# sanurielf/kvxopt

Measured on AMD Instinct MI355X. Metric: sparse Cholesky factor+solve GF/s, higher is better.
Workload: dtype f64; 1 GPU; 5-pt Laplacian 1000x1000, n=1000000, lower CCS int64, nrhs=1, factor+solve per step; nnz_lower=2998000, lnz=32346403, nsuper=58315, nlevels=18, max_front=1897, parallelism=1 GPU

## Files before the change

### kvxopt_amd/csrc/api.cpp

```cpp
#include "chol_internal.hpp"

#include <algorithm>
#include <chrono>
#include <climits>
#include <cstdio>
#include <cstdlib>
#include <cstring>
#include <stdexcept>
#include <string>
#include <mutex>
#include <vector>

using namespace kvx;

static thread_local std::string g_err;

namespace {
struct LazyRegistry {
    std::mutex mu;
    std::vector<std::shared_future<hipGraphExec_t>> futs;
    ~LazyRegistry()
    {
        std::lock_guard<std::mutex> lk(mu);
        for (auto &f : futs)
// ... 479 lines not shown
        destroy_graphs(F);
        lap("graphs");
        for (hipEvent_t e : F->prof_ev)
            if (e) pool_event_put(e, true);
        for (int i = 0; i < 3; i++) {
            if (F->side[i]) pool_stream_put(F->side[i]);
            if (F->ev_join[i]) pool_event_put(F->ev_join[i], false);
        }
        if (F->d_iperm) (void)pool_free(F->d_iperm);
        if (F->d_inv_ptr) (void)pool_free(F->d_inv_ptr);
        if (F->d_inv_src) (void)pool_free(F->d_inv_src);
        if (F->d_keep) (void)pool_free(F->d_keep);
        if (F->d_flists) (void)pool_free(F->d_flists);
        if (F->d_chain) (void)pool_free(F->d_chain);
        dist_release(F);
        for (void *p : {(void *)F->d_subs, (void *)F->d_subs_f, (void *)F->d_subs_lvl, (void *)F->d_cd_woff, (void *)F->d_lists_sw, (void *)F->d_depth})
            if (p) (void)pool_free(p);
        if (F->ev_fork) pool_event_put(F->ev_fork, false);
        for (hipEvent_t e : F->ev_u)
            if (e) pool_event_put(e, false);
        if (F->ev_ujoin) pool_event_put(F->ev_ujoin, false);
        for (hipEvent_t e : F->ev_lvl)
            if (e) pool_event_put(e, false);
        for (int i = 0; i < 4; i++)
            if (F->ev_pipe[i]) pool_event_put(F->ev_pipe[i], false);
        if (F->ev_in) pool_event_put(F->ev_in, false);
        if (F->ev_out) pool_event_put(F->ev_out, false);
        if (F->stream) pool_stream_put(F->stream);
        lap("streams");
    }
    delete F;
    lap("delete");
}

void kvx_free(void *p) { free(p); }

int kvx_dev_malloc(void **p, int64_t bytes) { HIPCHK(pool_malloc(p, (size_t)std::max<int64_t>(bytes, 1))); return KVX_OK; }
int kvx_dev_free(void *p) { HIPCHK(pool_free(p)); return KVX_OK; }
int kvx_dev_upload(void *dst, const void *src, int64_t bytes) { if (bytes > 0) HIPCHK(hipMemcpy(dst, src, (size_t)bytes, hipMemcpyHostToDevice)); return KVX_OK; }
int kvx_dev_download(void *dst, const void *src, int64_t bytes) { if (bytes > 0) HIPCHK(hipMemcpy(dst, src, (size_t)bytes, hipMemcpyDeviceToHost)); return KVX_OK; }
int kvx_dev_sync(void) { HIPCHK(hipDeviceSynchronize()); return KVX_OK; }
int kvx_dev_trim(void) { pool_release_all(); return KVX_OK; }
int kvx_dev_mem_info(int64_t *free_bytes, int64_t *total_bytes)
{
    size_t f = 0, t = 0;
    HIPCHK(hipMemGetInfo(&f, &t));
// ... 7 lines not shown
```

### kvxopt_amd/csrc/chol_factor.cpp

```cpp
#include "chol_internal.hpp"

#include <algorithm>
#include <climits>
#include <string>

namespace kvx {

int wait_for_caller(kvx_chol *F)
{
    HIPCHK(hipEventRecord(F->ev_in, nullptr));
    HIPCHK(hipStreamWaitEvent(F->stream, F->ev_in, 0));
    return KVX_OK;
}

namespace {

bool dbg_memset_nodes() { return getenv("KVX_DBG_MEMSET_NODES") != nullptr; }

int factor_prologue(kvx_chol *F)
{
    Symbolic &S = F->S;
    hipStream_t st = F->stream;
    const bool nodes = dbg_memset_nodes();
    if (F->d_scptr && !nodes) {
        ProfScope ps(F, FAM_SCATTER);
        launch_init_factor(st, F->d_Ax, F->d_ssrc, F->d_sdst, F->d_scptr, S.lsize, F->d_Lx, F->d_status);
        return KVX_OK;
    }
    if (nodes) {
        HIPCHK(hipMemsetAsync(F->d_Lx, 0, std::max<int64_t>(S.lsize, 1) * sizeof(double), st));
        HIPCHK(hipMemsetAsync(F->d_status, 0x7f, sizeof(int), st));
    } else {
        launch_clear_factor(st, F->d_Lx, S.lsize, F->d_status);
    }
    ProfScope ps(F, FAM_SCATTER);
    launch_scatter_a(st, F->d_Ax, F->d_amap, S.nnzA, F->d_Lx);
    return KVX_OK;
}

int factor_epilogue(kvx_chol *F)
{
    if (F->h_status_dev && !dbg_memset_nodes()) launch_publish_status(F->stream, F->d_status, F->h_status_dev);
    else HIPCHK(hipMemcpyAsync(F->h_status, F->d_status, sizeof(int), hipMemcpyDeviceToHost, F->stream));
    return KVX_OK;
}

int factor_subtree_walk(kvx_chol *F)
{
    hipStream_t st = F->stream;
    const int caps[3] = {32, 48, 64};
    hipStream_t ss[3] = {st, F->side[0], F->side[1]};
    const bool fork[3] = {false, F->nsubf[1] > 0, F->nsubf[2] > 0};
    if (fork[1] || fork[2]) {
        HIPCHK(hipEventRecord(F->ev_fork, st));
        for (int g = 1; g < 3; g++)
            if (fork[g]) HIPCHK(hipStreamWaitEvent(ss[g], F->ev_fork, 0));
    }
    const int64_t offs[3] = {0, F->nsubf[0], F->nsubf[0] + F->nsubf[1]};
    for (int g = 2; g >= 0; g--) {
        if (F->nsubf[g] == 0) continue;
        ProfScope ps(F, FAM_SMALL, ss[g]);
        launch_factor_subtree(ss[g], caps[g], F->ds, F->d_subs_f + offs[g], F->nsubf[g], F->d_depth, F->d_Lx, F->d_U[0], F->d_U[1], F->d_status);
    }
    for (int g = 1; g < 3; g++)
        if (fork[g]) { HIPCHK(hipEventRecord(F->ev_join[g - 1], ss[g])); HIPCHK(hipStreamWaitEvent(st, F->ev_join[g - 1], 0)); }
    return KVX_OK;
}

struct Level {
    kvx_chol *F;
    int l;
    const LevelPlan &P;
    const int32_t *lbase;
    const double *Uch;
    double *Uout;
    const int32_t *list;
    int nbig, bigm;
};

int small_fronts(const Level &L, bool side_used[2])
{
    kvx_chol *F = L.F;
    const LevelPlan &P = L.P;
    hipStream_t st = F->stream;
    const bool have_big = L.nbig > 0;
    struct Item { int c; int cnt; int64_t off; double est; int stream; int mcap; int kmax; };
    Item items[5];
    int nitems = 0;
    for (int c = KVX_CLS_LDS128; c < KVX_CLS_WAVE0; c++)
        if (P.cnt[c] > 0) {
            const double slots = c == KVX_CLS_LDS128 ? 512.0 : 1024.0;
            items[nitems++] = Item{c, P.cnt[c], P.off[c], (P.maxk[c] > 32 ? 80.0 : 45.0) * std::max(1.0, P.cnt[c] / slots), 0, 0, 0};
        }
    for (int c = KVX_CLS_WAVE0; c < KVX_NCLS; c += 2) {
        const int cnt = P.cnt[c] + P.cnt[c + 1];
        if (cnt == 0) continue;
        const int mcap = wave_class_mcap(c);
        const double base = mcap == 64 ? 35.0 : (mcap == 48 ? 28.0 : 18.0), slots = mcap == 64 ? 2048.0 : (mcap == 48 ? 4096.0 : 8192.0);
        items[nitems++] = Item{c, cnt, P.cnt[c] > 0 ? P.off[c] : P.off[c + 1], base * std::max(1.0, cnt / slots), 0, mcap, P.cnt[c] > 0 ? 32 : 16};
    }
// ... 69 lines not shown
{
    kvx_chol *F = L.F;
    hipStream_t st = F->stream;
    ProfScope ps(F, FAM_SYRK);
    if (cls) {
        const kvx_chol::ChainList &cl = F->chain_steps[(size_t)L.l][(size_t)(jb / KVX_NB)];
        launch_syrk_step(st, F->ds, F->d_chain + cl.off, F->chain_m.data() + cl.off, F->chain_k.data() + cl.off, cl.cnt, jb, klen,
                         F->d_Lx, L.Uout, F->d_Linv, F->d_status, col_lim);
    } else if (klen == 2 * KVX_NB) {
        launch_syrk_pair(st, F->ds, L.list, L.nbig, L.bigm, jb, F->d_Lx, L.Uout, F->d_Linv, F->d_status, col_lim);
    } else if (col_lim < KVX_COLS_PIVOT) {
        launch_syrk_inner(st, F->ds, L.list, L.nbig, L.bigm, jb, col_lim, F->d_Lx, L.Uout, F->d_Linv, F->d_status);
    } else {
        launch_syrk_trailing(st, F->ds, L.list, L.nbig, L.bigm, jb, F->d_Lx, L.Uout, F->d_Linv, F->d_status, col_lim);
    }
}

void trsm_step(const Level &L, int jb)
{
    ProfScope ps(L.F, FAM_TRSM);
    launch_trsm_blk(L.F->stream, L.F->ds, L.list, L.nbig, L.bigm, jb, L.F->d_Lx, L.F->d_Linv);
}

void chain_two_level(const Level &L)
{
    kvx_chol *F = L.F;
    hipStream_t st = F->stream;
    const int OB = F->K.outer_block, maxk = L.P.chain_maxk;
    for (int ob = 0; ob < maxk; ob += OB) {
        for (int jb = ob; jb < std::min(ob + OB, maxk); jb += KVX_NB) {
            trsm_step(L, jb);
            { ProfScope ps(F, FAM_SYRK); launch_syrk_inner(st, F->ds, L.list, L.nbig, L.bigm, jb, ob + OB, F->d_Lx, L.Uout, F->d_Linv, F->d_status); }
        }
        { ProfScope ps(F, FAM_SYRK); launch_syrk_outer(st, F->ds, L.list, L.nbig, L.bigm, ob, OB, F->d_Lx, L.Uout, F->d_Linv, F->d_status); }
    }
}

int chain_blocked(const Level &L)
{
    kvx_chol *F = L.F;
    hipStream_t st = F->stream;
    const int OB = F->K.u_block, maxk = L.P.chain_maxk;
    const std::vector<kvx_chol::ChainList> &far = F->u_steps[(size_t)L.l];
    hipStream_t su = (F->K.u_stream && F->prof_family < 0) ? F->side[2] : st;
    bool forked = false;
    for (int ob = 0, b = 0; ob < maxk; ob += OB, b++) {
        const int bend = std::min(ob + OB, maxk);
        for (int jb = ob; jb < bend; jb += KVX_NB) {
            trsm_step(L, jb);
            if (jb + KVX_NB < bend) syrk_step(L, true, jb, KVX_NB, ob + OB);
        }
        const kvx_chol::ChainList &fl = far[(size_t)b];
        if (fl.cnt > 0) {
            if (su != st) {
                while ((int)F->ev_u.size() <= 2 * b + 1) { hipEvent_t e = nullptr; HIPCHK(pool_event_get(&e, false)); F->ev_u.push_back(e); }
                HIPCHK(hipEventRecord(F->ev_u[(size_t)(2 * b)], st));
                HIPCHK(hipStreamWaitEvent(su, F->ev_u[(size_t)(2 * b)], 0));
                forked = true;
                syrk_count(SYRK_FAR_SIDE);
            }
            {
                ProfScope ps(F, FAM_SYRK, su);
                launch_syrk_far(su, F->ds, F->d_chain + fl.off, F->chain_m.data() + fl.off, F->chain_k.data() + fl.off, fl.cnt, ob, OB,
                                ob + 2 * OB, F->d_Lx, L.Uout);
            }
            if (su != st) HIPCHK(hipEventRecord(F->ev_u[(size_t)(2 * b + 1)], su));
        }
        if (bend < maxk) {
            if (su != st && b >= 1 && far[(size_t)(b - 1)].cnt > 0) HIPCHK(hipStreamWaitEvent(st, F->ev_u[(size_t)(2 * (b - 1) + 1)], 0));
            syrk_step(L, true, ob, OB, ob + 2 * OB);
        }
    }
    if (forked) {
        if (!F->ev_ujoin) HIPCHK(pool_event_get(&F->ev_ujoin, false));
        HIPCHK(hipEventRecord(F->ev_ujoin, su));
        HIPCHK(hipStreamWaitEvent(st, F->ev_ujoin, 0));
    }
    return KVX_OK;
}

void chain_pairs(const Level &L, bool cls)
{
    const int maxk = L.P.chain_maxk;
    for (int jb = 0; jb < maxk;) {
        const int64_t T = (L.bigm - jb - 1 + KVX_TILE - 1) / KVX_TILE;
        const bool pair = jb + KVX_NB < maxk && T * (T + 1) / 2 * L.nbig >= L.F->K.pair_tiles;
        trsm_step(L, jb);
        if (!pair) {
            syrk_step(L, cls, jb, KVX_NB, INT_MAX);
            jb += KVX_NB;
            continue;
        }
        syrk_step(L, cls, jb, KVX_NB, jb + 2 * KVX_NB);
        trsm_step(L, jb + KVX_NB);
        syrk_step(L, cls, jb, 2 * KVX_NB, INT_MAX);
        jb += 2 * KVX_NB;
    }
}

int pipe_level_hook(kvx_chol *F, int l)
{
    Symbolic &S = F->S;
    HIPCHK(hipEventRecord(F->ev_lvl[(size_t)l], F->stream));
    hipStream_t sw = F->K.pipe_own_stream ? F->side[2] : F->side[0];
    const SweepStreams ss2{sw, sw, sw, F->ev_pipe[1], F->ev_pipe[2], F->ev_pipe[3]};
    if (l == F->pipe_from) enqueue_fwd(F, F->d_X, S.n, F->pipe_nr, S.nlevels - 1, l, &ss2, true, true);
    else if (l < F->pipe_from) enqueue_fwd(F, F->d_X, S.n, F->pipe_nr, l, l, &ss2, true);
    return KVX_OK;
}

}

int enqueue_factor_body(kvx_chol *F, int lfrom, int lto, bool prologue, bool epilogue)
{
    Symbolic &S = F->S;
    int rc;
    if (prologue && (rc = factor_prologue(F))) return rc;
    if (lfrom < 0) lfrom = S.nlevels - 1;
    if (F->factor_subtrees && prologue && lfrom == S.nlevels - 1 && (rc = factor_subtree_walk(F))) return rc;
    const int32_t *lbase = F->fplan_on ? F->d_flists : F->d_lists;
    for (int l = lfrom; l >= lto; l--) {
        const LevelPlan &P = F->fplan_on ? F->fplan[l] : F->plan[l];
        const Level L{F, l, P, lbase, F->d_U[(l + 1) & 1], F->d_U[l & 1], lbase + P.off[KVX_CLS_BIG], P.cnt[KVX_CLS_BIG], P.maxm[KVX_CLS_BIG]};
        bool side_used[2];
        if ((rc = small_fronts(L, side_used))) return rc;
        if (L.nbig > 0) {
            assemble_big(L);
            const ChainChoice c = choose_chain(P, F->K, have_chain_lists(F, l, P));
            if (c.kind == CHAIN_TWO_LEVEL) chain_two_level(L);
            else if (c.kind == CHAIN_PAIRS) chain_pairs(L, c.cls);
            else if ((rc = chain_blocked(L))) return rc;
        }
        if ((rc = join_small_fronts(F, side_used))) return rc;
        if (F->pipe_on && (rc = pipe_level_hook(F, l))) return rc;
    }
    if (epilogue && (rc = factor_epilogue(F))) return rc;
    HIPCHK(hipGetLastError());
    return KVX_OK;
}

void dump_graph_dot(hipGraph_t graph)
{
    const char *dot = getenv("KVX_DBG_GRAPH_DOT");
    if (!dot) return;
    static int serial = 0;
    const std::string path = std::string(dot) + "." + std::to_string(serial++) + ".dot";
    if (hipGraphDebugDotPrint(graph, path.c_str(), 0) != hipSuccess) (void)hipGetLastError();
}

int enqueue_factor(kvx_chol *F)
{
    if (F->dist_nranks > 1) { set_err("sharded factor: use kvx_chol_dist_factorize"); return KVX_EINVAL; }
    hipStream_t st = F->stream;
    HIPCHK(hipEventRecord(F->ev[0], st));
    const char *dbg_ng = dbg_no_factor_graph();
    const bool graph_ok = F->K.use_graph && F->prof_family < 0 && !(dbg_ng && (atoll(dbg_ng) == 1 || atoll(dbg_ng) == F->S.n));
    F->factor_calls++;
    F->diag_valid = false;
    if (graph_ok && !F->g_factor.tried && F->factor_calls >= 2)
// ... 38 lines not shown
```

### kvxopt_amd/csrc/chol_internal.hpp

```cpp
#pragma once
#include "../../include/kvxhip.h"
#include "abi_guard.hpp"
#include "devpool.hpp"
#include "device.hpp"
#include "symbolic.hpp"

#include <chrono>
#include <cstdint>
#include <cstdlib>
#include <atomic>
#include <future>
#include <string>
#include <vector>

namespace kvx { void set_last_error(const std::string &s); struct DistState; }
#define set_err(s) ::kvx::set_last_error(s)
using namespace kvx;

#define HIPCHK(call)                                                                     \
    do {                                                                                 \
        hipError_t e_ = (call);                                                          \
        if (e_ != hipSuccess) {                                                          \
            set_err(std::string(#call) + ": " + hipGetErrorString(e_));                 \
            return KVX_EDEVICE;                                                          \
// ... 43 lines not shown
        tried = false;
    }
};

struct CholKnobs {
    int sub_maxf = 0;
    bool factor_subtrees = false;
    int u_block = 384;
    bool init_two_passes = false;
    bool use_subtrees = true;
    bool use_graph = true;
    int wide_from = -1;
    int side_spread = 1;
    int two_level_m = 6144;
    int outer_block = 1024;
    int64_t asm_potrf_wgs = 1024;
    int64_t pair_tiles = 3000;
    int defer_u = 1;
    bool syrk_direct = false;
    double blocked_gf = 0.5;
    int u_stream = 1;
    bool pipe_own_stream = false;
    bool solve_nofork = false;
};
CholKnobs read_chol_knobs();
inline const char *dbg_no_factor_graph() { return getenv("KVX_DBG_NO_FACTOR_GRAPH"); }

struct LevelPlan {
    int64_t off[KVX_NCLS];
    int cnt[KVX_NCLS];
    int maxm[KVX_NCLS];
    int maxk[KVX_NCLS];
    int big_maxk = 0;
    int chain_maxk = 0;
    double big_flops = 0.0;
    int64_t soff[3];
    int scnt[3];
    int smaxm[3];
};

struct kvx_chol {
    Symbolic S;
    kvx_chol_opts opts;
    CholKnobs K;
    bool dev_ready = false;
    bool numeric = false;
    bool pending = false;
    bool is_ll = true;
    double *d_diag = nullptr;
    bool diag_valid = false;
    int64_t minor = 0;
    hipStream_t stream = nullptr;
    hipStream_t side[3] = {nullptr, nullptr, nullptr};
    hipEvent_t ev_fork = nullptr, ev_join[3] = {nullptr, nullptr, nullptr};
    hipEvent_t ev_out = nullptr;
    hipEvent_t ev_in = nullptr;
    hipEvent_t ev[4] = {nullptr, nullptr, nullptr, nullptr};
    std::vector<hipEvent_t> ev_lvl;
    bool pipe_on = false;
    int pipe_nr = 0;
    int pipe_from = 0;
    hipEvent_t ev_pipe[4] = {nullptr, nullptr, nullptr, nullptr};
    SubDesc *d_subs_lvl = nullptr;
    std::vector<int> sub_lvl_off, sub_lvl_cnt;
    struct FusedGraph { int nrhs; double *B; int64_t ldB; int calls; LazyExec exec; };
    std::vector<FusedGraph> g_fused;
    bool have_ftime = false, have_stime = false;
    double ms_factor = 0, ms_solve = 0;

    int32_t *d_k = nullptr, *d_m = nullptr, *d_first = nullptr, *d_rowidx = nullptr, *d_rel = nullptr,
            *d_children = nullptr, *d_perm = nullptr, *d_lists = nullptr;
    int64_t *d_px = nullptr, *d_rowptr = nullptr, *d_ux = nullptr, *d_wx = nullptr, *d_childptr = nullptr,
            *d_amap = nullptr, *d_sdst = nullptr, *d_scptr = nullptr;
    double *d_Lx = nullptr, *d_U[2] = {nullptr, nullptr}, *d_Ax = nullptr;
    double *d_X = nullptr, *d_X0 = nullptr, *d_W[2] = {nullptr, nullptr}, *d_WK = nullptr;
    double *d_Linv = nullptr;
    int32_t *d_ssrc = nullptr;
    int64_t scnt = 0;
    int64_t *d_linv_off = nullptr;
    FrontDesc *d_fd = nullptr;
    ChildDesc *d_cd = nullptr;
    int32_t *d_tiles = nullptr;
// ... 82 lines not shown
};
enum { FAM_SCATTER = 0, FAM_SMALL = 1, FAM_ASSEMBLE = 2, FAM_POTRF = 3, FAM_TRSM = 4, FAM_SYRK = 5, FAM_FWD = 6, FAM_BWD = 7 };

inline void prof_collect(kvx_chol *F)
{
    for (size_t i = 0; i + 1 < F->prof_used; i += 2) {
        float ms = 0;
        if (hipEventElapsedTime(&ms, F->prof_ev[i], F->prof_ev[i + 1]) == hipSuccess) { F->prof_ms += ms; F->prof_launches++; }
    }
    F->prof_used = 0;
}


void build_plan_from(const Symbolic &S, const std::vector<int32_t> &lists, const std::vector<int64_t> &lptr, std::vector<LevelPlan> &plan);
void build_plan(kvx_chol *F);
int build_subtrees(kvx_chol *F);
int build_chain_lists(kvx_chol *F);
int ensure_device(kvx_chol *F);
int ensure_solve_ws(kvx_chol *F, int64_t nrhs);
int ensure_wide(kvx_chol *F);
void destroy_graphs(kvx_chol *F);
int wait_for_caller(kvx_chol *F);
int enqueue_factor_body(kvx_chol *F, int lfrom = -1, int lto = 0, bool prologue = true, bool epilogue = true);
int enqueue_factor(kvx_chol *F);
int finish_factor(kvx_chol *F, int64_t *minor);
void dump_graph_dot(hipGraph_t graph);
struct SweepStreams { hipStream_t main, lds, wave; hipEvent_t fork, join0, join1; };
void enqueue_fwd(kvx_chol *F, double *X, int64_t ldx, int nrhs, int lfrom = -1, int lto = 0, const SweepStreams *ss = nullptr, bool wait_levels = false,
                 bool sub_tail = false);
void enqueue_bwd(kvx_chol *F, double *X, int64_t ldx, int nrhs, int lfrom = 0, int lto = -1);
int solve_dev(kvx_chol *F, int sys, double *B, int64_t nrhs, int64_t ldB, bool async = false);
int factor_solve_dev(kvx_chol *F, const double *values_dev, double *B, int64_t nrhs, int64_t ldB, bool async = false);
int spsolve_forward_reach(kvx_chol *F, int sys, int64_t ncol, const int64_t *Bp, const int64_t *Bi, const double *Bx,
                          std::vector<int64_t> &xp, std::vector<int64_t> &xi, std::vector<double> &xx);
void dist_release(kvx_chol *F);

template <class Body>
void capture_graph(kvx_chol *F, Body body, LazyExec &out)
{
    out.tried = true;
    hipGraph_t graph = nullptr;
    if (hipStreamBeginCapture(F->stream, hipStreamCaptureModeRelaxed) != hipSuccess) { (void)hipGetLastError(); return; }
    int rc = body();
    hipError_t e = hipStreamEndCapture(F->stream, &graph);
    if (rc != KVX_OK || e != hipSuccess || !graph) { (void)hipGetLastError(); if (graph) (void)hipGraphDestroy(graph); return; }
    dump_graph_dot(graph);
// ... 19 lines not shown
```

### kvxopt_amd/csrc/chol_setup.cpp

```cpp
#include "chol_internal.hpp"

#include <algorithm>
#include <climits>
#include <vector>

namespace kvx {

bool syrk_direct() { static const bool v = [] { const char *e = getenv("KVX_SYRK_DIRECT"); return e && e[0] == '1'; }(); return v; }

CholKnobs read_chol_knobs()
{
    CholKnobs K;
    const char *e;
    auto is1 = [](const char *v) { return v && v[0] == '1'; };
    if ((e = getenv("KVX_SUB_MAXF"))) K.sub_maxf = std::max(1, std::min(atoi(e), KVX_SUB_MAXF));
    K.factor_subtrees = is1(getenv("KVX_FACTOR_SUBTREES"));
    if ((e = getenv("KVX_U_BLOCK"))) K.u_block = std::max(64, atoi(e) / 64 * 64);
    K.init_two_passes = getenv("KVX_INIT_TWO_PASSES") != nullptr;
    K.use_subtrees = !is1(getenv("KVX_NO_SUBTREES"));
    K.use_graph = !is1(getenv("KVX_NO_GRAPH"));
    if ((e = getenv("KVX_WIDE_FROM"))) K.wide_from = std::max(0, atoi(e));
    if ((e = getenv("KVX_SIDE_SPREAD"))) K.side_spread = atoi(e);
    if ((e = getenv("KVX_TWO_LEVEL_M"))) K.two_level_m = atoi(e);
    if ((e = getenv("KVX_OUTER_BLOCK")) && atoi(e) >= 64) K.outer_block = atoi(e) / 64 * 64;
    if ((e = getenv("KVX_ASM_POTRF_WGS"))) K.asm_potrf_wgs = atoll(e);
    if ((e = getenv("KVX_PAIR_TILES"))) K.pair_tiles = atoll(e);
    if ((e = getenv("KVX_DEFER_U"))) K.defer_u = atoi(e);
    K.syrk_direct = syrk_direct();
    if ((e = getenv("KVX_BLOCKED_GF"))) K.blocked_gf = atof(e);
    if ((e = getenv("KVX_U_STREAM"))) K.u_stream = atoi(e);
    K.pipe_own_stream = is1(getenv("KVX_PIPE_OWN_STREAM"));
    K.solve_nofork = (e = getenv("KVX_SOLVE_NOFORK")) && atoi(e) != 0;
    return K;
}

void build_plan_from(const Symbolic &S, const std::vector<int32_t> &lists, const std::vector<int64_t> &lptr, std::vector<LevelPlan> &plan)
{
    plan.assign((size_t)S.nlevels, LevelPlan());
    for (int l = 0; l < S.nlevels; l++) {
        LevelPlan &P = plan[l];
        for (int c = 0; c < KVX_NCLS; c++) { P.off[c] = 0; P.cnt[c] = 0; P.maxm[c] = 0; P.maxk[c] = 0; }
        for (int g = 0; g < 3; g++) { P.soff[g] = 0; P.scnt[g] = 0; P.smaxm[g] = 0; }
        for (int64_t q = lptr[l]; q < lptr[l + 1]; q++) {
            int s = lists[q];
            int m = S.sn_m[s], k = S.sn_k[s];
            int c = front_class(m, k);
            if (P.cnt[c] == 0) P.off[c] = q;
            P.cnt[c]++;
            P.maxm[c] = std::max(P.maxm[c], m);
            P.maxk[c] = std::max(P.maxk[c], k);
            if (c == KVX_CLS_BIG) {
                P.big_maxk = std::max(P.big_maxk, k);
                P.chain_maxk = std::max(P.chain_maxk, k);
                P.big_flops += (double)k * k * k / 3.0 + (double)(m - k) * k * (double)m;
            }
// ... 395 lines not shown
```

### kvxopt_amd/csrc/chol_solve.cpp

```cpp
#include "chol_internal.hpp"

#include <algorithm>
#include <chrono>
#include <climits>
#include <cstdio>
#include <vector>

namespace kvx {

struct LevelStreams {
    SweepStreams S;
    hipStream_t lds, wave;
    bool fork_lds, fork_wave;
    static SweepStreams own(kvx_chol *F)
    {
        if (F->K.solve_nofork) return SweepStreams{F->stream, F->stream, F->stream, F->ev_fork, F->ev_join[0], F->ev_join[1]};
        return SweepStreams{F->stream, F->side[0], F->side[1], F->ev_fork, F->ev_join[0], F->ev_join[1]};
    }
    LevelStreams(kvx_chol *F, bool have_big, bool have_lds, bool have_wave, const SweepStreams *ss = nullptr) : S(ss ? *ss : own(F))
    {
        fork_lds = have_lds && (have_big || have_wave) && S.lds != S.main;
        fork_wave = have_wave && have_big && S.wave != S.main;
        lds = fork_lds ? S.lds : S.main;
        wave = fork_wave ? S.wave : S.main;
// ... 316 lines not shown
        for (auto &e : F->ev_lvl) HIPCHK(pool_event_get(&e, false));
        for (int i = 0; i < 4; i++) HIPCHK(pool_event_get(&F->ev_pipe[i], false));
        if (F->nsub > 0) {
            std::vector<std::vector<SubDesc>> by((size_t)S.nlevels);
            for (const SubDesc &d : F->subs_host) by[(size_t)S.depth[(size_t)d.hi]].push_back(d);
            std::vector<SubDesc> flat;
            F->sub_lvl_off.assign((size_t)S.nlevels, 0);
            F->sub_lvl_cnt.assign((size_t)S.nlevels, 0);
            for (int l = 0; l < S.nlevels; l++) {
                F->sub_lvl_off[(size_t)l] = (int)flat.size();
                F->sub_lvl_cnt[(size_t)l] = (int)by[(size_t)l].size();
                flat.insert(flat.end(), by[(size_t)l].begin(), by[(size_t)l].end());
            }
            if (F->d_subs_lvl) { (void)pool_free(F->d_subs_lvl); F->d_subs_lvl = nullptr; }
            if ((rc = upload(&F->d_subs_lvl, flat))) return rc;
        }
        int lim = 4;
        if (const char *e = getenv("KVX_PIPE_FRONTS")) lim = atoi(e);
        F->pipe_from = 0;
        for (int l = 0; l < S.nlevels; l++) {
            if (S.levelptr[(size_t)l + 1] - S.levelptr[(size_t)l] > lim) break;
            F->pipe_from = l;
        }
    }
    lap("pipeline set-up");
    hipStream_t st = F->stream, s2 = F->K.pipe_own_stream ? F->side[2] : F->side[0];
    auto body = [&]() -> int {
        HIPCHK(hipEventRecord(F->ev_pipe[0], st));
        HIPCHK(hipStreamWaitEvent(s2, F->ev_pipe[0], 0));
        launch_perm_gather(s2, F->d_perm, n, nr, B, ldB, F->d_X, n);
        launch_copy_d(s2, F->d_X0, F->d_X, n * (int64_t)nr);
        F->pipe_on = true;
        F->pipe_nr = nr;
        const int rb = enqueue_factor_body(F);
        F->pipe_on = false;
        if (rb) return rb;
        HIPCHK(hipEventRecord(F->ev_pipe[0], s2));
        HIPCHK(hipStreamWaitEvent(st, F->ev_pipe[0], 0));
        enqueue_bwd(F, F->d_X, n, nr);
        launch_perm_scatter(st, F->d_perm, n, nr, F->d_X, n, B, ldB);
        return hipGetLastError() == hipSuccess ? KVX_OK : KVX_EDEVICE;
    };
    HIPCHK(hipEventRecord(F->ev[0], st));
    F->factor_calls++;
    F->diag_valid = false;
    kvx_chol::FusedGraph *slot = nullptr;
    if (F->K.use_graph && !dbg_no_factor_graph() && !getenv("KVX_FUSED_EAGER")) {
        for (auto &g : F->g_fused)
            if (g.nrhs == nr && g.B == B && g.ldB == ldB) slot = &g;
        if (!slot) {
            if (F->g_fused.size() >= 4) {
                for (auto &g : F->g_fused) g.exec.drop();
                F->g_fused.clear();
            }
            F->g_fused.push_back({nr, B, ldB, 0, LazyExec{}});
            slot = &F->g_fused.back();
        }
    }
    if ((rc = capture_or_replay(F, slot, true, body))) return rc;
    lap("capture, graph launch or eager enqueue");
    HIPCHK(hipEventRecord(F->ev[1], st));
    HIPCHK(hipGetLastError());
    F->pending = true;
// ... 174 lines not shown
```

### kvxopt_amd/csrc/device.hpp

```cpp
#pragma once
#include <hip/hip_runtime.h>
#include <cstdint>
#include <utility>

namespace kvx {

struct DevSym {
    const int32_t *k;
    const int32_t *m;
    const int32_t *first;
    const int64_t *px;
    const int64_t *rowptr;
    const int32_t *rowidx;
    const int32_t *rel;
    const int64_t *ux;
    const int64_t *wx;
    const int64_t *childptr;
    const int32_t *children;
    const int64_t *linv;
    const struct FrontDesc *fd;
    const struct ChildDesc *cd;
    const int32_t *tiles;
    double piv_floor, piv_repl;
};
// ... 170 lines not shown
void launch_fwd_level(hipStream_t st, const DevSym &ds, const int32_t *list, int count, int max_m,
                      const double *Lx, double *X, int64_t ldx, int nrhs,
                      const double *Wchild, double *Wout, int64_t wstride);
void launch_bwd_level(hipStream_t st, const DevSym &ds, const int32_t *list, int count, int max_m,
                      const double *Lx, double *X, int64_t ldx, int nrhs);
void launch_fwd_wave(hipStream_t st, const DevSym &ds, const int32_t *list, int count, int kmax,
                     const double *Lx, double *X, int64_t ldx, int nrhs, const double *Wchild, double *Wout, int64_t wstride);
void launch_bwd_wave(hipStream_t st, const DevSym &ds, const int32_t *list, int count, int mcap, int kmax,
                     const double *Lx, double *X, int64_t ldx, int nrhs);
void launch_fwd_subtree(hipStream_t st, const DevSym &ds, const SubDesc *subs, int nsub, const int32_t *edges,
                        const double *Lx, double *X, int64_t ldx, int nrhs, double *W0, double *W1, int64_t wstride,
                        const int32_t *depth);
void launch_bwd_subtree(hipStream_t st, const DevSym &ds, const SubDesc *subs, int nsub, int nsub32, const double *Lx, double *X,
                        int64_t ldx, int nrhs);
void launch_bwd_subtree_group(hipStream_t st, int mcap, const DevSym &ds, const SubDesc *subs, int count, const double *Lx, double *X,
                              int64_t ldx);
void launch_fwd_lds(hipStream_t st, const DevSym &ds, const int32_t *list, int count, int kmax,
                    const double *Lx, double *X, int64_t ldx, int nrhs, const double *Wchild, double *Wout, int64_t wstride);
void launch_bwd_lds(hipStream_t st, const DevSym &ds, const int32_t *list, int count,
                    const double *Lx, double *X, int64_t ldx, int nrhs);
void launch_fwd_big(hipStream_t st, const DevSym &ds, const int32_t *list, int count, int max_m, int max_k,
                    const double *Lx, const double *Linv, double *X, const double *X0, int64_t ldx, int nrhs,
                    double *WK, int64_t ldw, const double *Wchild, double *Wout, int64_t wstride, int level_count = 0);
void launch_bwd_big(hipStream_t st, const DevSym &ds, const int32_t *list, int count, int max_m, int max_k,
                    const double *Lx, const double *Linv, double *X, int64_t ldx, int nrhs, double *WK, int64_t ldw);
void launch_perm_gather(hipStream_t st, const int32_t *perm, int64_t n, int nrhs, const double *in, int64_t ldi,
                        double *out, int64_t ldo);
void launch_perm_scatter(hipStream_t st, const int32_t *perm, int64_t n, int nrhs, const double *in, int64_t ldi,
                         double *out, int64_t ldo);
void launch_wide_gather(hipStream_t st, const int32_t *iperm, int64_t n, int nrhs, const double *B, int64_t ldB, double *XT,
                        const double *diag, int mode);
void launch_wide_scatter(hipStream_t st, const int32_t *iperm, int64_t n, int nrhs, const double *XT, double *B, int64_t ldB,
                         const double *diag, int mode);
void launch_wide_fwd_small(hipStream_t st, const DevSym &ds, const int32_t *list, int count, int kmax, int nchunk, const double *Lx,
                           double *XT, int64_t n, const double *Wch, double *Wout, int64_t wstride, const int32_t *inv_ptr,
                           const int32_t *inv_src);
void launch_wide_bwd_small(hipStream_t st, const DevSym &ds, const int32_t *list, int count, int kmax, int nchunk, const double *Lx,
                           double *XT, int64_t n);
void launch_wide_fwd_big(hipStream_t st, const DevSym &ds, const int32_t *list, int count, int max_m, int max_k, int nchunk,
                         const double *Lx, const double *Linv, double *XT, int64_t n, const double *Wch, double *Wout,
                         int64_t wstride, const int32_t *inv_ptr, const int32_t *inv_src);
void launch_wide_bwd_big(hipStream_t st, const DevSym &ds, const int32_t *list, int count, int max_k, int nchunk, const double *Lx,
                         const double *Linv, double *XT, int64_t n);
void launch_zero_slots(hipStream_t st, const int64_t *slots, int count, int nrhs, double *W, int64_t wstride);
void launch_scatter_entries(hipStream_t st, const int64_t *pos, const double *val, int64_t count, double *X);
void launch_mask_rows(hipStream_t st, const uint8_t *keep, int64_t n, int nrhs, double *X, int64_t ldx);
// ... 5 lines not shown
```

### kvxopt_amd/csrc/kernels_big.hip

```cpp
#include "device.hpp"
#include "tile_classes.hpp"

#include <algorithm>
#include <atomic>
#include <climits>
#include <cstdint>
#include <cstdlib>
#include <type_traits>
#include <utility>

namespace kvx {

typedef double d4 __attribute__((ext_vector_type(4)));

#ifdef KVX_PHASE_TIMING
__device__ unsigned long long g_phase[16];
#define KVX_STAMP(var) const unsigned long long var = __builtin_readcyclecounter()
#define KVX_PHASE_ADD(slot, a, b) do { if (threadIdx.x == 0) atomicAdd(&g_phase[slot], (unsigned long long)((b) - (a))); } while (0)
#else
#define KVX_STAMP(var) do { } while (0)
#define KVX_PHASE_ADD(slot, a, b) do { } while (0)
#endif
constexpr int NB = KVX_NB;

// ... 979 lines not shown
    syrk_count(SYRK_T64_GRID);
    hipLaunchKernelGGL(k_syrk_trailing<64>, dim3(T, TC, (unsigned)count), dim3(256), 0, st, ds, list, jb, Lx, Uout, Linv, status, ob_end, no_classes());
}

void launch_syrk_outer(hipStream_t st, const DevSym &ds, const int32_t *list, int count, int max_m, int ob, int ob_len,
                       double *Lx, double *Uout, double *Linv, int *status)
{
    if (count <= 0) return;
    int rows = max_m - ob - 1;
    if (rows <= 0) return;
    syrk_count(SYRK_OUTER);
    hipLaunchKernelGGL(k_syrk_trailing128<false>, syrk128_grid(rows, count), dim3(512), 0, st, ds, list, ob, ob_len, Lx, Uout, Linv, status, ColOwner{1, 1, 0, 0, INT_MAX, 0});
}

void launch_syrk_outer_dist(hipStream_t st, const DevSym &ds, const int32_t *list, int max_m, int ob, int ob_len,
                            int own_ob, int own_g, int own_r, int c_from, int c_to, double *Lx, double *Uout)
{
    int rows = max_m - ob - 1;
    if (rows <= 0 || c_from >= c_to) return;
    hipLaunchKernelGGL(k_syrk_trailing128<true>, syrk128_grid(rows, 1), dim3(512), 0, st, ds, list, ob, ob_len, Lx, Uout,
                       (double *)nullptr, (int *)nullptr, ColOwner{own_ob, own_g, own_r, c_from, c_to, 0});
}

constexpr int SB = 256;
constexpr int SOLVE_NT = 1024;

__device__ __forceinline__ constexpr int sblk(int ib, int s) { return ib * (ib - 1) / 2 + s; }

template <bool FIRST, int ROWS>
__global__ __launch_bounds__(SOLVE_NT) void k_fwd_big_step(DevSym ds, const int32_t *__restrict__ list, int jb0,
                                                           const double *__restrict__ Lx, const double *__restrict__ Linv,
                                                           double *__restrict__ X, const double *__restrict__ X0, int64_t ldx,
                                                           double *__restrict__ WK, int64_t ldw,
                                                           const double *__restrict__ Wc,
                                                           double *__restrict__ Wo, int64_t wstride)
{
    unsigned bx, by, rh;
    kvx_part_front_rhs(bx, by, rh);
    __shared__ double red[3 * 16 * NB];
    __shared__ double own[FIRST ? ROWS : 1];
    __shared__ double wsh[SB];
    __shared__ double ysh[SB];
    const FrontDesc fd = ds.fd[list[by]];
    const int k = fd.k, m = fd.m, f = fd.first, tid = threadIdx.x;
    if (jb0 >= k) return;
    const int nb = min(SB, k - jb0);
    const int rbase = jb0 + nb + bx * ROWS;
// ... 543 lines not shown
#pragma unroll
        for (int c = 0; c < 4; c++)
#pragma unroll
            for (int j = 0; j < 4; j++)
                v[c][j] = kvx_ld0(P, (int64_t)(jb0 + lane + j * NB) + (int64_t)(c0 + c) * m, lane + j * NB < nb && c0 + c < jb0);
#pragma unroll
        for (int b = 0; b < RB; b++) {
            if (b < nv) {
                double a[4] = {0.0, 0.0, 0.0, 0.0};
#pragma unroll
                for (int c = 0; c < 4; c++)
#pragma unroll
                    for (int j = 0; j < 4; j++) a[c] = __builtin_fma(v[c][j], xsh[b][lane + j * NB], a[c]);
                const double u = wave_sum4(a[0], a[1], a[2], a[3], lane);
                if (lane < 4 && c0 + o < jb0) WK[(int64_t)(r0 + b) * ldw + f + c0 + o] -= u;
            }
        }
    }
}

constexpr int KVX_BIG_RB = 8;
constexpr int KVX_BIG_MR_FROM = 64;

void launch_fwd_big(hipStream_t st, const DevSym &ds, const int32_t *list, int count, int max_m, int max_k,
                    const double *Lx, const double *Linv, double *X, const double *X0, int64_t ldx, int nrhs,
                    double *WK, int64_t ldw, const double *Wchild, double *Wout, int64_t wstride, int level_count)
{
    if (count <= 0 || nrhs <= 0) return;
    static const int narrow_wgs = [] { const char *e = getenv("KVX_FWD_NARROW_WGS"); return e ? atoi(e) : 512; }();
    if (nrhs >= KVX_BIG_MR_FROM) {
        for (int jb = 0; jb < max_k; jb += SB) {
            int rows = max_m - jb - 1;
            if ((int64_t)std::max(1, (rows + 63) / 64) * std::max(level_count, count) <= narrow_wgs) {
                dim3 grid((unsigned)std::max(1, (rows + 63) / 64), (unsigned)count, (unsigned)nrhs);
                if (jb == 0) hipLaunchKernelGGL((k_fwd_big_step<true, 64>), grid, dim3(SOLVE_NT), 0, st, ds, list, jb, Lx, Linv, X, X0, ldx, WK, ldw, Wchild, Wout, wstride);
                else hipLaunchKernelGGL((k_fwd_big_step<false, 64>), grid, dim3(SOLVE_NT), 0, st, ds, list, jb, Lx, Linv, X, X0, ldx, WK, ldw, Wchild, Wout, wstride);
                continue;
            }
            const unsigned gz = (unsigned)((nrhs + KVX_BIG_RB - 1) / KVX_BIG_RB);
            dim3 g1(1, (unsigned)count, gz), g2((unsigned)std::max(1, (rows + 255) / 256), (unsigned)count, gz);
            if (jb == 0) {
                hipLaunchKernelGGL((k_fwd_big_step_mr<true, KVX_BIG_RB, 1>), g1, dim3(SOLVE_NT), 0, st, ds, list, jb, Lx, Linv, X, X0, ldx, nrhs, WK, ldw, Wchild, Wout, wstride);
                hipLaunchKernelGGL((k_fwd_big_step_mr<true, KVX_BIG_RB, 2>), g2, dim3(SOLVE_NT), 0, st, ds, list, jb, Lx, Linv, X, X0, ldx, nrhs, WK, ldw, Wchild, Wout, wstride);
            } else {
                hipLaunchKernelGGL((k_fwd_big_step_mr<false, KVX_BIG_RB, 1>), g1, dim3(SOLVE_NT), 0, st, ds, list, jb, Lx, Linv, X, X0, ldx, nrhs, WK, ldw, Wchild, Wout, wstride);
                hipLaunchKernelGGL((k_fwd_big_step_mr<false, KVX_BIG_RB, 2>), g2, dim3(SOLVE_NT), 0, st, ds, list, jb, Lx, Linv, X, X0, ldx, nrhs, WK, ldw, Wchild, Wout, wstride);
            }
        }
        return;
    }
    for (int jb = 0; jb < max_k; jb += SB) {
        int rows = max_m - jb - 1;
        const int64_t wg64 = (int64_t)std::max(1, (rows + 63) / 64) * std::max(level_count, count);
        const bool narrow = wg64 <= narrow_wgs;
        dim3 grid((unsigned)std::max(1, narrow ? (rows + 63) / 64 : (rows + 255) / 256), (unsigned)count, (unsigned)nrhs);
        if (jb == 0) {
            if (narrow) hipLaunchKernelGGL((k_fwd_big_step<true, 64>), grid, dim3(SOLVE_NT), 0, st, ds, list, jb, Lx, Linv, X, X0, ldx, WK, ldw, Wchild, Wout, wstride);
            else hipLaunchKernelGGL((k_fwd_big_step<true, 256>), grid, dim3(SOLVE_NT), 0, st, ds, list, jb, Lx, Linv, X, X0, ldx, WK, ldw, Wchild, Wout, wstride);
        } else {
            if (narrow) hipLaunchKernelGGL((k_fwd_big_step<false, 64>), grid, dim3(SOLVE_NT), 0, st, ds, list, jb, Lx, Linv, X, X0, ldx, WK, ldw, Wchild, Wout, wstride);
            else hipLaunchKernelGGL((k_fwd_big_step<false, 256>), grid, dim3(SOLVE_NT), 0, st, ds, list, jb, Lx, Linv, X, X0, ldx, WK, ldw, Wchild, Wout, wstride);
        }
    }
}

void launch_bwd_big(hipStream_t st, const DevSym &ds, const int32_t *list, int count, int max_m, int max_k,
                    const double *Lx, const double *Linv, double *X, int64_t ldx, int nrhs, double *WK, int64_t ldw)
{
    if (count <= 0 || nrhs <= 0) return;
    (void)max_m;
    if (nrhs >= KVX_BIG_MR_FROM) {
        const unsigned gz = (unsigned)((nrhs + KVX_BIG_RB - 1) / KVX_BIG_RB);
        hipLaunchKernelGGL((k_bwd_big_init_mr<KVX_BIG_RB>), dim3((unsigned)((max_k + 3) / 4), (unsigned)count, gz), dim3(256), 0, st,
                           ds, list, Lx, X, ldx, nrhs, WK, ldw);
        for (int b = (max_k + SB - 1) / SB - 1; b >= 0; b--) {
            hipLaunchKernelGGL((k_bwd_big_step_mr<KVX_BIG_RB, 1>), dim3(1, (unsigned)count, gz), dim3(SOLVE_NT), 0, st, ds, list, b, Lx, Linv,
                               X, ldx, nrhs, WK, ldw);
            if (b > 0)
                hipLaunchKernelGGL((k_bwd_big_step_mr<KVX_BIG_RB, 2>), dim3((unsigned)(b * SB / NB), (unsigned)count, gz), dim3(SOLVE_NT), 0, st, ds, list, b, Lx, Linv,
                                   X, ldx, nrhs, WK, ldw);
        }
        return;
    }
    hipLaunchKernelGGL(k_bwd_big_init, dim3((unsigned)((max_k + 3) / 4), (unsigned)count, (unsigned)nrhs), dim3(256), 0, st,
                       ds, list, Lx, X, ldx, WK, ldw);
    for (int b = (max_k + SB - 1) / SB - 1; b >= 0; b--) {
// ... 8 lines not shown
```

Baseline: 2318 GF/s.

## Pipeline root-front forward solve per block and defer level sweeps behind factor

Splits the forward solve of the root level into per-256-column block launches, each gated by an event recorded after the matching trsm step of the root factorization. The solve can then start on the side stream while the trailing SYRK updates of the root front are still running. It also defers each level's sweep until after the next level's assembly, and moves the status publish onto the sweep stream. The cost is more events and launches, plus more complex ordering logic that could hurt if the side-stream work competes with factor kernels.

```diff
diff --git a/kvxopt_amd/csrc/api.cpp b/kvxopt_amd/csrc/api.cpp
--- a/kvxopt_amd/csrc/api.cpp
+++ b/kvxopt_amd/csrc/api.cpp
@@ -525,6 +525,9 @@
         if (F->ev_ujoin) pool_event_put(F->ev_ujoin, false);
         for (hipEvent_t e : F->ev_lvl)
             if (e) pool_event_put(e, false);
+        for (hipEvent_t e : F->ev_blk)
+            if (e) pool_event_put(e, false);
+        if (F->ev_stat) pool_event_put(F->ev_stat, false);
         for (int i = 0; i < 4; i++)
             if (F->ev_pipe[i]) pool_event_put(F->ev_pipe[i], false);
         if (F->ev_in) pool_event_put(F->ev_in, false);
diff --git a/kvxopt_amd/csrc/chol_factor.cpp b/kvxopt_amd/csrc/chol_factor.cpp
--- a/kvxopt_amd/csrc/chol_factor.cpp
+++ b/kvxopt_amd/csrc/chol_factor.cpp
@@ -35,13 +35,6 @@
     }
     ProfScope ps(F, FAM_SCATTER);
     launch_scatter_a(st, F->d_Ax, F->d_amap, S.nnzA, F->d_Lx);
-    return KVX_OK;
-}
-
-int factor_epilogue(kvx_chol *F)
-{
-    if (F->h_status_dev && !dbg_memset_nodes()) launch_publish_status(F->stream, F->d_status, F->h_status_dev);
-    else HIPCHK(hipMemcpyAsync(F->h_status, F->d_status, sizeof(int), hipMemcpyDeviceToHost, F->stream));
     return KVX_OK;
 }
 
@@ -76,6 +69,7 @@
     double *Uout;
     const int32_t *list;
     int nbig, bigm;
+    bool blocks;
 };
 
 int small_fronts(const Level &L, bool side_used[2])
@@ -191,6 +185,37 @@
     launch_trsm_blk(L.F->stream, L.F->ds, L.list, L.nbig, L.bigm, jb, L.F->d_Lx, L.F->d_Linv);
 }
 
+hipStream_t sweep_stream(const kvx_chol *F) { return F->K.pipe_own_stream ? F->side[2] : F->side[0]; }
+
+int root_block_flush(kvx_chol *F)
+{
+    const int j = F->pend_blk;
+    if (j < 0) return KVX_OK;
+    F->pend_blk = -1;
+    const Symbolic &S = F->S;
+    const LevelPlan &P = F->plan[0];
+    hipStream_t sw = sweep_stream(F);
+    HIPCHK(hipStreamWaitEvent(sw, F->ev_blk[(size_t)j], 0));
+    launch_fwd_big_step(sw, F->ds, F->d_lists + P.soff[0], P.scnt[0], P.smaxm[0], j * KVX_SOLVE_SB, F->d_Lx, F->d_Linv, F->d_X, F->d_X0, S.n,
+                        F->pipe_nr, F->d_WK, S.n, F->d_W[1], F->d_W[0], std::max(S.wrk_size[0], S.wrk_size[1]), P.scnt[0]);
+    return KVX_OK;
+}
+
+int root_block_hook(const Level &L, int jb)
+{
+    kvx_chol *F = L.F;
+    if (!L.blocks) return KVX_OK;
+    const bool last = jb + KVX_NB >= L.P.chain_maxk;
+    if (!last && (jb + KVX_NB) % KVX_SOLVE_SB != 0) return KVX_OK;
+    if (int rc = root_block_flush(F)) return rc;
+    const int j = jb / KVX_SOLVE_SB;
+    if ((size_t)j >= F->ev_blk.size()) { set_err("root pipeline: block event out of range"); return KVX_EINVAL; }
+    HIPCHK(hipEventRecord(F->ev_blk[(size_t)j], F->stream));
+    F->pend_blk = j;
+    if (!(F->K.pipe_edge_order & 1)) return root_block_flush(F);
+    return KVX_OK;
+}
+
 void chain_two_level(const Level &L)
 {
     kvx_chol *F = L.F;
@@ -217,7 +242,11 @@
         const int bend = std::min(ob + OB, maxk);
         for (int jb = ob; jb < bend; jb += KVX_NB) {
             trsm_step(L, jb);
-            if (jb + KVX_NB < bend) syrk_step(L, true, jb, KVX_NB, ob + OB);
+            if (int rc = root_block_hook(L, jb)) return rc;
+            if (jb + KVX_NB < bend) {
+                syrk_step(L, true, jb, KVX_NB, ob + OB);
+                if (int rc = root_block_flush(F)) return rc;
+            }
         }
         const kvx_chol::ChainList &fl = far[(size_t)b];
         if (fl.cnt > 0) {
@@ -238,8 +267,10 @@
         if (bend < maxk) {
             if (su != st && b >= 1 && far[(size_t)(b - 1)].cnt > 0) HIPCHK(hipStreamWaitEvent(st, F->ev_u[(size_t)(2 * (b - 1) + 1)], 0));
             syrk_step(L, true, ob, OB, ob + 2 * OB);
-        }
-    }
+            if (int rc = root_block_flush(F)) return rc;
+        }
+    }
+    if (int rc = root_block_flush(F)) return rc;
     if (forked) {
         if (!F->ev_ujoin) HIPCHK(pool_event_get(&F->ev_ujoin, false));
         HIPCHK(hipEventRecord(F->ev_ujoin, su));
@@ -248,30 +279,52 @@
     return KVX_OK;
 }
 
-void chain_pairs(const Level &L, bool cls)
+int chain_pairs(const Level &L, bool cls)
 {
     const int maxk = L.P.chain_maxk;
     for (int jb = 0; jb < maxk;) {
         const int64_t T = (L.bigm - jb - 1 + KVX_TILE - 1) / KVX_TILE;
         const bool pair = jb + KVX_NB < maxk && T * (T + 1) / 2 * L.nbig >= L.F->K.pair_tiles;
         trsm_step(L, jb);
+        if (int rc = root_block_hook(L, jb)) return rc;
         if (!pair) {
             syrk_step(L, cls, jb, KVX_NB, INT_MAX);
+            if (int rc = root_block_flush(L.F)) return rc;
             jb += KVX_NB;
             continue;
         }
         syrk_step(L, cls, jb, KVX_NB, jb + 2 * KVX_NB);
+        if (int rc = root_block_flush(L.F)) return rc;
         trsm_step(L, jb + KVX_NB);
+        if (int rc = root_block_hook(L, jb + KVX_NB)) return rc;
         syrk_step(L, cls, jb, 2 * KVX_NB, INT_MAX);
+        if (int rc = root_block_flush(L.F)) return rc;
         jb += 2 * KVX_NB;
     }
-}
-
-int pipe_level_hook(kvx_chol *F, int l)
+    return root_block_flush(L.F);
+}
+
+int pipe_level_sweep(kvx_chol *F, int l);
+int pipe_level_hook(kvx_chol *F, int l, bool swept)
+{
+    HIPCHK(hipEventRecord(F->ev_lvl[(size_t)l], F->stream));
+    if (swept) return KVX_OK;
+    if ((F->K.pipe_edge_order & 2) && l > 0) { F->pend_lvl = l; return KVX_OK; }
+    return pipe_level_sweep(F, l);
+}
+
+int pipe_level_flush(kvx_chol *F)
+{
+    const int l = F->pend_lvl;
+    if (l < 0) return KVX_OK;
+    F->pend_lvl = -1;
+    return pipe_level_sweep(F, l);
+}
+
+int pipe_level_sweep(kvx_chol *F, int l)
 {
     Symbolic &S = F->S;
-    HIPCHK(hipEventRecord(F->ev_lvl[(size_t)l], F->stream));
-    hipStream_t sw = F->K.pipe_own_stream ? F->side[2] : F->side[0];
+    hipStream_t sw = sweep_stream(F);
     const SweepStreams ss2{sw, sw, sw, F->ev_pipe[1], F->ev_pipe[2], F->ev_pipe[3]};
     if (l == F->pipe_from) enqueue_fwd(F, F->d_X, S.n, F->pipe_nr, S.nlevels - 1, l, &ss2, true, true);
     else if (l < F->pipe_from) enqueue_fwd(F, F->d_X, S.n, F->pipe_nr, l, l, &ss2, true);
@@ -280,30 +333,41 @@
 
 }
 
+int factor_epilogue(kvx_chol *F, hipStream_t st)
+{
+    if (F->h_status_dev && !dbg_memset_nodes()) launch_publish_status(st, F->d_status, F->h_status_dev);
+    else HIPCHK(hipMemcpyAsync(F->h_status, F->d_status, sizeof(int), hipMemcpyDeviceToHost, st));
+    return KVX_OK;
+}
+
 int enqueue_factor_body(kvx_chol *F, int lfrom, int lto, bool prologue, bool epilogue)
 {
     Symbolic &S = F->S;
     int rc;
+    F->pend_blk = F->pend_lvl = -1;
     if (prologue && (rc = factor_prologue(F))) return rc;
     if (lfrom < 0) lfrom = S.nlevels - 1;
     if (F->factor_subtrees && prologue && lfrom == S.nlevels - 1 && (rc = factor_subtree_walk(F))) return rc;
     const int32_t *lbase = F->fplan_on ? F->d_flists : F->d_lists;
     for (int l = lfrom; l >= lto; l--) {
         const LevelPlan &P = F->fplan_on ? F->fplan[l] : F->plan[l];
-        const Level L{F, l, P, lbase, F->d_U[(l + 1) & 1], F->d_U[l & 1], lbase + P.off[KVX_CLS_BIG], P.cnt[KVX_CLS_BIG], P.maxm[KVX_CLS_BIG]};
+        Level L{F, l, P, lbase, F->d_U[(l + 1) & 1], F->d_U[l & 1], lbase + P.off[KVX_CLS_BIG], P.cnt[KVX_CLS_BIG], P.maxm[KVX_CLS_BIG], false};
         bool side_used[2];
         if ((rc = small_fronts(L, side_used))) return rc;
         if (L.nbig > 0) {
             assemble_big(L);
+            if (F->pipe_on && (rc = pipe_level_flush(F))) return rc;
             const ChainChoice c = choose_chain(P, F->K, have_chain_lists(F, l, P));
+            L.blocks = F->pipe_on && F->pipe_blocks && l == 0 && c.kind != CHAIN_TWO_LEVEL;
             if (c.kind == CHAIN_TWO_LEVEL) chain_two_level(L);
-            else if (c.kind == CHAIN_PAIRS) chain_pairs(L, c.cls);
-            else if ((rc = chain_blocked(L))) return rc;
+            else if (c.kind == CHAIN_PAIRS) rc = chain_pairs(L, c.cls);
+            else rc = chain_blocked(L);
+            if (rc) return rc;
         }
         if ((rc = join_small_fronts(F, side_used))) return rc;
-        if (F->pipe_on && (rc = pipe_level_hook(F, l))) return rc;
-    }
-    if (epilogue && (rc = factor_epilogue(F))) return rc;
+        if (F->pipe_on && ((rc = pipe_level_flush(F)) || (rc = pipe_level_hook(F, l, L.blocks)))) return rc;
+    }
+    if (epilogue && (rc = factor_epilogue(F, F->stream))) return rc;
     HIPCHK(hipGetLastError());
     return KVX_OK;
 }
diff --git a/kvxopt_amd/csrc/chol_internal.hpp b/kvxopt_amd/csrc/chol_internal.hpp
--- a/kvxopt_amd/csrc/chol_internal.hpp
+++ b/kvxopt_amd/csrc/chol_internal.hpp
@@ -89,6 +89,9 @@
     int u_stream = 1;
     bool pipe_own_stream = false;
     bool solve_nofork = false;
+    int pipe_blocks = 1;
+    int pipe_edge_order = 3;
+    int status_side = 1;
 };
 CholKnobs read_chol_knobs();
 inline const char *dbg_no_factor_graph() { return getenv("KVX_DBG_NO_FACTOR_GRAPH"); }
@@ -125,6 +128,10 @@
     hipEvent_t ev[4] = {nullptr, nullptr, nullptr, nullptr};
     std::vector<hipEvent_t> ev_lvl;
     bool pipe_on = false;
+    bool pipe_blocks = false;
+    std::vector<hipEvent_t> ev_blk;
+    int pend_blk = -1, pend_lvl = -1;
+    hipEvent_t ev_stat = nullptr;
     int pipe_nr = 0;
     int pipe_from = 0;
     hipEvent_t ev_pipe[4] = {nullptr, nullptr, nullptr, nullptr};
@@ -253,6 +260,7 @@
 void destroy_graphs(kvx_chol *F);
 int wait_for_caller(kvx_chol *F);
 int enqueue_factor_body(kvx_chol *F, int lfrom = -1, int lto = 0, bool prologue = true, bool epilogue = true);
+int factor_epilogue(kvx_chol *F, hipStream_t st);
 int enqueue_factor(kvx_chol *F);
 int finish_factor(kvx_chol *F, int64_t *minor);
 void dump_graph_dot(hipGraph_t graph);
diff --git a/kvxopt_amd/csrc/chol_setup.cpp b/kvxopt_amd/csrc/chol_setup.cpp
--- a/kvxopt_amd/csrc/chol_setup.cpp
+++ b/kvxopt_amd/csrc/chol_setup.cpp
@@ -31,6 +31,9 @@
     if ((e = getenv("KVX_U_STREAM"))) K.u_stream = atoi(e);
     K.pipe_own_stream = is1(getenv("KVX_PIPE_OWN_STREAM"));
     K.solve_nofork = (e = getenv("KVX_SOLVE_NOFORK")) && atoi(e) != 0;
+    if ((e = getenv("KVX_PIPE_BLOCKS"))) K.pipe_blocks = atoi(e);
+    if ((e = getenv("KVX_STATUS_SIDE"))) K.status_side = atoi(e);
+    if ((e = getenv("KVX_PIPE_EDGE_ORDER"))) K.pipe_edge_order = atoi(e);
     return K;
 }
 
diff --git a/kvxopt_amd/csrc/chol_solve.cpp b/kvxopt_amd/csrc/chol_solve.cpp
--- a/kvxopt_amd/csrc/chol_solve.cpp
+++ b/kvxopt_amd/csrc/chol_solve.cpp
@@ -362,6 +362,14 @@
             if (S.levelptr[(size_t)l + 1] - S.levelptr[(size_t)l] > lim) break;
             F->pipe_from = l;
         }
+        const LevelPlan &P0 = F->plan[0];
+        F->pipe_blocks = F->K.pipe_blocks != 0 && !F->fplan_on && P0.scnt[0] > 0 && F->sw_cnt[0] == 0 && (F->solve_merged || P0.scnt[1] == 0) &&
+                         (F->nsub == 0 || F->sub_lvl_cnt[0] == 0) && (F->pipe_from > 0 || S.nlevels == 1);
+        if (F->pipe_blocks) {
+            F->ev_blk.assign((size_t)((P0.big_maxk + KVX_SOLVE_SB - 1) / KVX_SOLVE_SB), nullptr);
+            for (auto &e : F->ev_blk) HIPCHK(pool_event_get(&e, false));
+        }
+        HIPCHK(pool_event_get(&F->ev_stat, false));
     }
     lap("pipeline set-up");
     hipStream_t st = F->stream, s2 = F->K.pipe_own_stream ? F->side[2] : F->side[0];
@@ -372,13 +380,21 @@
         launch_copy_d(s2, F->d_X0, F->d_X, n * (int64_t)nr);
         F->pipe_on = true;
         F->pipe_nr = nr;
-        const int rb = enqueue_factor_body(F);
+        const bool stat_side = F->K.status_side != 0;
+        const int rb = enqueue_factor_body(F, -1, 0, true, !stat_side);
         F->pipe_on = false;
         if (rb) return rb;
         HIPCHK(hipEventRecord(F->ev_pipe[0], s2));
         HIPCHK(hipStreamWaitEvent(st, F->ev_pipe[0], 0));
+        if (stat_side) {
+            int rs;
+            HIPCHK(hipStreamWaitEvent(s2, F->ev_lvl[0], 0));
+            if ((rs = factor_epilogue(F, s2))) return rs;
+            HIPCHK(hipEventRecord(F->ev_stat, s2));
+        }
         enqueue_bwd(F, F->d_X, n, nr);
         launch_perm_scatter(st, F->d_perm, n, nr, F->d_X, n, B, ldB);
+        if (stat_side) HIPCHK(hipStreamWaitEvent(st, F->ev_stat, 0));
         return hipGetLastError() == hipSuccess ? KVX_OK : KVX_EDEVICE;
     };
     HIPCHK(hipEventRecord(F->ev[0], st));
diff --git a/kvxopt_amd/csrc/device.hpp b/kvxopt_amd/csrc/device.hpp
--- a/kvxopt_amd/csrc/device.hpp
+++ b/kvxopt_amd/csrc/device.hpp
@@ -216,6 +216,10 @@
 void launch_fwd_big(hipStream_t st, const DevSym &ds, const int32_t *list, int count, int max_m, int max_k,
                     const double *Lx, const double *Linv, double *X, const double *X0, int64_t ldx, int nrhs,
                     double *WK, int64_t ldw, const double *Wchild, double *Wout, int64_t wstride, int level_count = 0);
+constexpr int KVX_SOLVE_SB = 256;
+void launch_fwd_big_step(hipStream_t st, const DevSym &ds, const int32_t *list, int count, int max_m, int jb,
+                         const double *Lx, const double *Linv, double *X, const double *X0, int64_t ldx, int nrhs,
+                         double *WK, int64_t ldw, const double *Wchild, double *Wout, int64_t wstride, int level_count);
 void launch_bwd_big(hipStream_t st, const DevSym &ds, const int32_t *list, int count, int max_m, int max_k,
                     const double *Lx, const double *Linv, double *X, int64_t ldx, int nrhs, double *WK, int64_t ldw);
 void launch_perm_gather(hipStream_t st, const int32_t *perm, int64_t n, int nrhs, const double *in, int64_t ldi,
diff --git a/kvxopt_amd/csrc/kernels_big.hip b/kvxopt_amd/csrc/kernels_big.hip
--- a/kvxopt_amd/csrc/kernels_big.hip
+++ b/kvxopt_amd/csrc/kernels_big.hip
@@ -1025,7 +1025,7 @@
                        (double *)nullptr, (int *)nullptr, ColOwner{own_ob, own_g, own_r, c_from, c_to, 0});
 }
 
-constexpr int SB = 256;
+constexpr int SB = KVX_SOLVE_SB;
 constexpr int SOLVE_NT = 1024;
 
 __device__ __forceinline__ constexpr int sblk(int ib, int s) { return ib * (ib - 1) / 2 + s; }
@@ -1615,46 +1615,43 @@
 constexpr int KVX_BIG_RB = 8;
 constexpr int KVX_BIG_MR_FROM = 64;
 
+void launch_fwd_big_step(hipStream_t st, const DevSym &ds, const int32_t *list, int count, int max_m, int jb,
+                         const double *Lx, const double *Linv, double *X, const double *X0, int64_t ldx, int nrhs,
+                         double *WK, int64_t ldw, const double *Wchild, double *Wout, int64_t wstride, int level_count)
+{
+    if (count <= 0 || nrhs <= 0) return;
+    static const int narrow_wgs = [] { const char *e = getenv("KVX_FWD_NARROW_WGS"); return e ? atoi(e) : 512; }();
+    const int rows = max_m - jb - 1;
+    const int64_t wg64 = (int64_t)std::max(1, (rows + 63) / 64) * std::max(level_count, count);
+    const bool narrow = wg64 <= narrow_wgs;
+    if (nrhs >= KVX_BIG_MR_FROM && !narrow) {
+        const unsigned gz = (unsigned)((nrhs + KVX_BIG_RB - 1) / KVX_BIG_RB);
+        dim3 g1(1, (unsigned)count, gz), g2((unsigned)std::max(1, (rows + 255) / 256), (unsigned)count, gz);
+        if (jb == 0) {
+            hipLaunchKernelGGL((k_fwd_big_step_mr<true, KVX_BIG_RB, 1>), g1, dim3(SOLVE_NT), 0, st, ds, list, jb, Lx, Linv, X, X0, ldx, nrhs, WK, ldw, Wchild, Wout, wstride);
+            hipLaunchKernelGGL((k_fwd_big_step_mr<true, KVX_BIG_RB, 2>), g2, dim3(SOLVE_NT), 0, st, ds, list, jb, Lx, Linv, X, X0, ldx, nrhs, WK, ldw, Wchild, Wout, wstride);
+        } else {
+            hipLaunchKernelGGL((k_fwd_big_step_mr<false, KVX_BIG_RB, 1>), g1, dim3(SOLVE_NT), 0, st, ds, list, jb, Lx, Linv, X, X0, ldx, nrhs, WK, ldw, Wchild, Wout, wstride);
+            hipLaunchKernelGGL((k_fwd_big_step_mr<false, KVX_BIG_RB, 2>), g2, dim3(SOLVE_NT), 0, st, ds, list, jb, Lx, Linv, X, X0, ldx, nrhs, WK, ldw, Wchild, Wout, wstride);
+        }
+        return;
+    }
+    dim3 grid((unsigned)std::max(1, narrow ? (rows + 63) / 64 : (rows + 255) / 256), (unsigned)count, (unsigned)nrhs);
+    if (jb == 0) {
+        if (narrow) hipLaunchKernelGGL((k_fwd_big_step<true, 64>), grid, dim3(SOLVE_NT), 0, st, ds, list, jb, Lx, Linv, X, X0, ldx, WK, ldw, Wchild, Wout, wstride);
+        else hipLaunchKernelGGL((k_fwd_big_step<true, 256>), grid, dim3(SOLVE_NT), 0, st, ds, list, jb, Lx, Linv, X, X0, ldx, WK, ldw, Wchild, Wout, wstride);
+    } else {
+        if (narrow) hipLaunchKernelGGL((k_fwd_big_step<false, 64>), grid, dim3(SOLVE_NT), 0, st, ds, list, jb, Lx, Linv, X, X0, ldx, WK, ldw, Wchild, Wout, wstride);
+        else hipLaunchKernelGGL((k_fwd_big_step<false, 256>), grid, dim3(SOLVE_NT), 0, st, ds, list, jb, Lx, Linv, X, X0, ldx, WK, ldw, Wchild, Wout, wstride);
+    }
+}
+
 void launch_fwd_big(hipStream_t st, const DevSym &ds, const int32_t *list, int count, int max_m, int max_k,
                     const double *Lx, const double *Linv, double *X, const double *X0, int64_t ldx, int nrhs,
                     double *WK, int64_t ldw, const double *Wchild, double *Wout, int64_t wstride, int level_count)
 {
-    if (count <= 0 || nrhs <= 0) return;
-    static const int narrow_wgs = [] { const char *e = getenv("KVX_FWD_NARROW_WGS"); return e ? atoi(e) : 512; }();
-    if (nrhs >= KVX_BIG_MR_FROM) {
-        for (int jb = 0; jb < max_k; jb += SB) {
-            int rows = max_m - jb - 1;
-            if ((int64_t)std::max(1, (rows + 63) / 64) * std::max(level_count, count) <= narrow_wgs) {
-                dim3 grid((unsigned)std::max(1, (rows + 63) / 64), (unsigned)count, (unsigned)nrhs);
-                if (jb == 0) hipLaunchKernelGGL((k_fwd_big_step<true, 64>), grid, dim3(SOLVE_NT), 0, st, ds, list, jb, Lx, Linv, X, X0, ldx, WK, ldw, Wchild, Wout, wstride);
-                else hipLaunchKernelGGL((k_fwd_big_step<false, 64>), grid, dim3(SOLVE_NT), 0, st, ds, list, jb, Lx, Linv, X, X0, ldx, WK, ldw, Wchild, Wout, wstride);
-                continue;
-            }
-            const unsigned gz = (unsigned)((nrhs + KVX_BIG_RB - 1) / KVX_BIG_RB);
-            dim3 g1(1, (unsigned)count, gz), g2((unsigned)std::max(1, (rows + 255) / 256), (unsigned)count, gz);
-            if (jb == 0) {
-                hipLaunchKernelGGL((k_fwd_big_step_mr<true, KVX_BIG_RB, 1>), g1, dim3(SOLVE_NT), 0, st, ds, list, jb, Lx, Linv, X, X0, ldx, nrhs, WK, ldw, Wchild, Wout, wstride);
-                hipLaunchKernelGGL((k_fwd_big_step_mr<true, KVX_BIG_RB, 2>), g2, dim3(SOLVE_NT), 0, st, ds, list, jb, Lx, Linv, X, X0, ldx, nrhs, WK, ldw, Wchild, Wout, wstride);
-            } else {
-                hipLaunchKernelGGL((k_fwd_big_step_mr<false, KVX_BIG_RB, 1>), g1, dim3(SOLVE_NT), 0, st, ds, list, jb, Lx, Linv, X, X0, ldx, nrhs, WK, ldw, Wchild, Wout, wstride);
-                hipLaunchKernelGGL((k_fwd_big_step_mr<false, KVX_BIG_RB, 2>), g2, dim3(SOLVE_NT), 0, st, ds, list, jb, Lx, Linv, X, X0, ldx, nrhs, WK, ldw, Wchild, Wout, wstride);
-            }
-        }
-        return;
-    }
-    for (int jb = 0; jb < max_k; jb += SB) {
-        int rows = max_m - jb - 1;
-        const int64_t wg64 = (int64_t)std::max(1, (rows + 63) / 64) * std::max(level_count, count);
-        const bool narrow = wg64 <= narrow_wgs;
-        dim3 grid((unsigned)std::max(1, narrow ? (rows + 63) / 64 : (rows + 255) / 256), (unsigned)count, (unsigned)nrhs);
-        if (jb == 0) {
-            if (narrow) hipLaunchKernelGGL((k_fwd_big_step<true, 64>), grid, dim3(SOLVE_NT), 0, st, ds, list, jb, Lx, Linv, X, X0, ldx, WK, ldw, Wchild, Wout, wstride);
-            else hipLaunchKernelGGL((k_fwd_big_step<true, 256>), grid, dim3(SOLVE_NT), 0, st, ds, list, jb, Lx, Linv, X, X0, ldx, WK, ldw, Wchild, Wout, wstride);
-        } else {
-            if (narrow) hipLaunchKernelGGL((k_fwd_big_step<false, 64>), grid, dim3(SOLVE_NT), 0, st, ds, list, jb, Lx, Linv, X, X0, ldx, WK, ldw, Wchild, Wout, wstride);
-            else hipLaunchKernelGGL((k_fwd_big_step<false, 256>), grid, dim3(SOLVE_NT), 0, st, ds, list, jb, Lx, Linv, X, X0, ldx, WK, ldw, Wchild, Wout, wstride);
-        }
-    }
+    for (int jb = 0; jb < max_k; jb += SB)
+        launch_fwd_big_step(st, ds, list, count, max_m, jb, Lx, Linv, X, X0, ldx, nrhs, WK, ldw, Wchild, Wout, wstride, level_count);
 }
 
 void launch_bwd_big(hipStream_t st, const DevSym &ds, const int32_t *list, int count, int max_m, int max_k,
```

Measured after the change: 2288 GF/s. 0.987x the previous value.
